# rlabbe/filterpy

Hardware: NVIDIA H100
Metric: kf_predict_update_filter_steps_per_sec (higher is better)
Workload: dtype f32

## Files before the change

filterpy_b200/csrc/kf_fast.cu:

```cuda
#include <string.h>
#include "bke_internal.cuh"
#include "kf_regtile.cuh"
#include "ptx.cuh"

namespace bke {
namespace {

__device__ __forceinline__ void st_hint(float *addr, float4 v, uint64_t pol)
{
    asm volatile("st.global.L2::cache_hint.v4.f32 [%0], {%1, %2, %3, %4}, %5;"
                 ::"l"(addr), "f"(v.x), "f"(v.y), "f"(v.z), "f"(v.w), "l"(pol) : "memory");
}

__device__ __forceinline__ uint32_t ld_relaxed_gpu(const uint32_t *addr)
{
    uint32_t v;
    asm volatile("ld.relaxed.gpu.global.u32 %0, [%1];" : "=r"(v) : "l"(addr) : "memory");
    return v;
}
__device__ __forceinline__ uint32_t atom_add_acq_rel_gpu(uint32_t *addr, uint32_t v)
{
    uint32_t old;
    asm volatile("atom.add.acq_rel.gpu.global.u32 %0, [%1], %2;" : "=r"(old) : "l"(addr), "r"(v) : "memory");
    return old;
}

constexpr int TILE = 128;

constexpr int SYM_Q_PLANES = 10, SYM_PLANES = 13;

constexpr int WORDS = BKE_KF42_MODEL_WORDS, W_F = 0, W_Q = 16, W_H = 26, W_R = 34;
constexpr uint64_t PREDICT_WORDS = (1ull << W_H) - 1;
constexpr int REC_RUNS = (WORDS + 1) / 2;
constexpr int q_word(int i, int j)
{
    const int r = i < j ? i : j, c = i < j ? j : i;
    return W_Q + r * 4 - r * (r - 1) / 2 + (c - r);
}

template <uint64_t Z, uint64_t O>
struct WordPattern {
    static constexpr uint64_t ZERO = Z, ONE = O;
    static constexpr bool any = (ZERO | ONE) != 0;
    static constexpr bool structural(int e) { return ((Z | O) >> e) & 1; }
    static constexpr uint32_t F0(int i) { return (uint32_t)(Z >> (W_F + 4 * i)) & 15u; }
    static constexpr uint32_t F1(int i) { return (uint32_t)(O >> (W_F + 4 * i)) & 15u; }
    static constexpr uint32_t H0(int a) { return (uint32_t)(Z >> (W_H + 4 * a)) & 15u; }
    static constexpr uint32_t H1(int a) { return (uint32_t)(O >> (W_H + 4 * a)) & 15u; }
    static constexpr bool Q0(int i, int j) { return (Z >> q_word(i, j)) & 1; }
    static constexpr bool R0(int a, int b) { return (Z >> (W_R + a + b)) & 1; }
};
struct NoPattern : WordPattern<0, 0> {};
struct Cv2dPattern : WordPattern<
    (1ull << 2) | (1ull << 3) | (1ull << 4) | (1ull << 6) | (1ull << 7) | (1ull << 8) | (1ull << 9) | (1ull << 12) |
        (1ull << 13) | (1ull << 14) | (1ull << q_word(0, 2)) | (1ull << q_word(0, 3)) | (1ull << q_word(1, 2)) |
        (1ull << q_word(1, 3)) | (1ull << 27) | (1ull << 28) | (1ull << 29) | (1ull << 30) | (1ull << 31) |
        (1ull << 33) | (1ull << (W_R + 1)),
    (1ull << 0) | (1ull << 5) | (1ull << 10) | (1ull << 15) | (1ull << 26) | (1ull << 32)> {};

template <typename T, int N, int M, bool SHARED = false, int REC = 0, int ZS = 1>
struct Stage {
    static constexpr int XB = TILE * N * sizeof(T);
    static constexpr int PB = TILE * N * N * sizeof(T);
    static constexpr int HB = TILE * M * N * sizeof(T);
    static constexpr int RB = TILE * M * M * sizeof(T);
    static constexpr int ZB = TILE * M * sizeof(T);
    static constexpr int QB = REC == 1 ? TILE * SYM_PLANES * sizeof(T) : REC == 2 ? TILE * WORDS * sizeof(T) : PB;
    static constexpr int align_up(int v) { return (v + 127) & ~127; }
    static constexpr int OP = 0;
    static constexpr int OF = OP + align_up(PB);
    static constexpr int OQ = OF + (SHARED || REC == 2 ? 0 : align_up(PB));
    static constexpr int OH = OQ + (SHARED ? 0 : align_up(QB));
    static constexpr int OX = OH + (SHARED || REC == 2 ? 0 : align_up(HB));
    static constexpr int OR_ = OX + align_up(XB);
    static constexpr int OZ = OR_ + (SHARED || REC ? 0 : align_up(RB));
    static constexpr int BYTES = OZ + ZS * align_up(ZB);
};

template <int ROWB>
__device__ __forceinline__ float4 lds_chunk(const unsigned char *base, int row, int c)
{
    return *reinterpret_cast<const float4 *>(base + row * ROWB + c * 16);
}

template <int ROWS>
__device__ __forceinline__ void lds_row(const unsigned char *base, int row, float (&m)[ROWS][4])
{
    const int r = (row / (8 / ROWS)) & (ROWS - 1);
    float4 v[ROWS];
#pragma unroll
    for (int c = 0; c < ROWS; c++)
        v[c] = *reinterpret_cast<const float4 *>(base + row * ROWS * 16 + ((c + r) & (ROWS - 1)) * 16);
#pragma unroll
    for (int step = 1; step < ROWS; step <<= 1) {
        const bool rot = r & step;
        float4 w[ROWS];
#pragma unroll
        for (int i = 0; i < ROWS; i++) {
            const float4 a = v[i], b = v[(i - step) & (ROWS - 1)];
            w[i] = make_float4(rot ? b.x : a.x, rot ? b.y : a.y, rot ? b.z : a.z, rot ? b.w : a.w);
        }
#pragma unroll
        for (int i = 0; i < ROWS; i++) v[i] = w[i];
    }
#pragma unroll
    for (int i = 0; i < ROWS; i++) { m[i][0] = v[i].x; m[i][1] = v[i].y; m[i][2] = v[i].z; m[i][3] = v[i].w; }
}

template <int N, int M>
struct FastP {
    int64_t N_filters;
    int num_tiles;
    int l2_hints;
    int reverse;
    float alpha_sq;
    const float *x, *P, *z;
    const float *F, *Q, *H, *R;
    const float *rec;
    float Fh[N * N], Qh[N * N], Hh[M * N], Rh[M * M];
    float *x_out, *P_out;
    const uint8_t *valid;
    float *x_prior, *P_prior, *K, *y, *S, *SI, *ll;
    int32_t *status;
    int sticky;
    uint64_t varying;
    int slot_off[WORDS];
    int rec_planes;
    int rec_copy;
    int rec_runs;
    int run_first[REC_RUNS], run_len[REC_RUNS];
    const float *zs[BKE_KF42_MAX_RING];
    int n_steps;
    int ring_ox, ring_oz, ring_stage;
    uint32_t *order;
};

constexpr int STAGES = 2;
constexpr int kf42_ctas_per_sm(int shared, int ring = 0) { return ring ? 4 : shared == 2 ? 5 : (shared ? 4 : 3); }

template <int MODE, int SHARED, bool EXTRAS, int REC = 0, int RING = 0, class PAT = NoPattern>
__global__ void __launch_bounds__(TILE, kf42_ctas_per_sm(SHARED, RING))
kf42_f32_kernel(const __grid_constant__ FastP<4, 2> p)
{
    constexpr int N = 4, M = 2;
    static_assert(!(REC && SHARED), "the packed records hold per-filter models");
    static_assert(!RING || (MODE == 3 && REC == 2 && !EXTRAS), "the fused ring steps the packed model words");
    static_assert(!PAT::any || RING, "a pattern instance is a fused ring");
    constexpr int ZS = RING ? RING : 1;
    using St = Stage<float, N, M, SHARED != 0, REC, ZS>;
    constexpr int SYM_FIRST = (MODE & 1) ? 0 : SYM_Q_PLANES;
    constexpr int SYM_LAST = (MODE & 2) ? SYM_PLANES : SYM_Q_PLANES;
    constexpr uint32_t SYM_BYTES = (SYM_LAST - SYM_FIRST) * TILE * 4;
    constexpr bool DO_P = MODE & 1, DO_U = MODE & 2;
    extern __shared__ __align__(128) unsigned char smem[];
    __shared__ __align__(8) uint64_t full[STAGES];

    const int tid = threadIdx.x;
    const int stage_bytes = RING ? p.ring_stage : St::BYTES, off_x = RING ? p.ring_ox : St::OX,
              off_z = RING ? p.ring_oz : St::OZ;

    const uint64_t pol_first = policy_evict_first(), pol_last = policy_evict_last();
    auto issue = [&](int tile, int stage) {
        unsigned char *sb = smem + stage * stage_bytes;
        uint64_t *bar = &full[stage];
        const int64_t f0 = (int64_t)tile * TILE;
        const int64_t left = p.N_filters - f0;
        const uint32_t nf = left < TILE ? (uint32_t)left : (uint32_t)TILE;
        const uint32_t zb = (nf * M * 4) & ~15u;
        uint32_t tx = nf * (N + N * N) * 4;
        if (!SHARED && REC != 2 && DO_P) tx += nf * (REC ? 1 : 2) * N * N * 4;
        if (!SHARED && REC != 2 && DO_U) tx += nf * (M * N + (REC ? 0 : M * M)) * 4;
        if (REC == 1) tx += SYM_BYTES;
        if (REC == 2) tx += (uint32_t)p.rec_copy * TILE * 4;
        if (DO_U) tx += RING ? p.n_steps * zb : zb;
        mbar_expect_tx(bar, tx);
        auto load = [&](int off, const float *src, int per_filter, uint32_t bytes, uint64_t pol) {
            if (p.l2_hints) bulk_load_hint(sb + off, src + f0 * per_filter, bytes, bar, pol);
            else bulk_load(sb + off, src + f0 * per_filter, bytes, bar);
        };
        load(St::OP, p.P, N * N, nf * N * N * 4, pol_last);
        load(off_x, p.x, N, nf * N * 4, pol_last);
        if (!SHARED && REC != 2 && DO_P) {
            load(St::OF, p.F, N * N, nf * N * N * 4, pol_first);
            if (!REC) load(St::OQ, p.Q, N * N, nf * N * N * 4, pol_first);
        }
        if (!SHARED && REC != 2 && DO_U) {
            load(St::OH, p.H, M * N, nf * M * N * 4, pol_first);
            if (!REC) load(St::OR_, p.R, M * M, nf * M * M * 4, pol_first);
        }
        if (REC == 1) load(St::OQ + SYM_FIRST * TILE * 4, p.rec + SYM_FIRST * TILE, SYM_PLANES, SYM_BYTES, pol_first);
        if (REC == 2)
            for (int r = 0; r < p.rec_runs; r++)
                load(St::OQ + p.run_first[r] * TILE * 4, p.rec + p.run_first[r] * TILE, p.rec_planes,
                     p.run_len[r] * TILE * 4, pol_first);
        if (!RING && DO_U && zb) load(St::OZ, p.z, M, zb, pol_first);
        if (RING && zb)
            for (int k = 0; k < p.n_steps; k++) load(off_z + k * St::align_up(St::ZB), p.zs[k], M, zb, pol_first);
    };

    if (tid == 0) {
        for (int s = 0; s < STAGES; s++) mbar_init(&full[s], 1);
        fence_mbar_init();
    }
    float F[N][N], Q[N][N], H[M][N], R[M][M];
    if (SHARED == 2) {
#pragma unroll
        for (int i = 0; i < N; i++)
#pragma unroll
            for (int j = 0; j < N; j++) { F[i][j] = p.Fh[i * N + j]; Q[i][j] = p.Qh[i * N + j]; }
#pragma unroll
        for (int a = 0; a < M; a++) {
#pragma unroll
            for (int j = 0; j < N; j++) H[a][j] = p.Hh[a * N + j];
#pragma unroll
            for (int b = 0; b < M; b++) R[a][b] = p.Rh[a * M + b];
        }
    }
    griddep_wait();
    __shared__ uint32_t order_epoch;
    if (RING && p.order && tid == 0) order_epoch = ld_relaxed_gpu(p.order);
    __syncthreads();
    const int reverse = RING && p.order ? (int)(order_epoch & 1u) : p.reverse;
    const int base = reverse ? p.num_tiles - 1 : 0, sign = reverse ? -1 : 1;
    if (tid == 0) {
        for (int s = 0; s < STAGES; s++) {
            int tile = blockIdx.x + s * gridDim.x;
            if (tile < p.num_tiles) issue(base + sign * tile, s);
        }
    }
    if (SHARED == 1) {
        if (DO_P) {
#pragma unroll
            for (int i = 0; i < N; i++)
#pragma unroll
                for (int j = 0; j < N; j++) { F[i][j] = __ldg(p.F + i * N + j); Q[i][j] = __ldg(p.Q + i * N + j); }
        }
        if (DO_U) {
#pragma unroll
            for (int a = 0; a < M; a++) {
#pragma unroll
                for (int j = 0; j < N; j++) H[a][j] = __ldg(p.H + a * N + j);
#pragma unroll
                for (int b = 0; b < M; b++) R[a][b] = __ldg(p.R + a * M + b);
            }
        }
    }

    int it = 0;
    for (int tile = blockIdx.x; tile < p.num_tiles; tile += gridDim.x, it++) {
        const int stage = it % STAGES;
        const uint32_t parity = (it / STAGES) & 1;
        const unsigned char *sb = smem + stage * stage_bytes;
        mbar_wait(&full[stage], parity);

        float x[N], P[N][N], z[ZS][M];
        {
            float4 v = lds_chunk<16>(sb + off_x, tid, 0);
            x[0] = v.x; x[1] = v.y; x[2] = v.z; x[3] = v.w;
        }
        lds_row<N>(sb + St::OP, tid, P);
        const unsigned char *rec = sb + St::OQ + tid * 4;
        auto word = [&](int e, float shared) -> float {
            if (PAT::structural(e)) return (PAT::ONE >> e) & 1 ? 1.f : 0.f;
            if (REC == 1) return *reinterpret_cast<const float *>(rec + (e < W_H ? e - W_Q : e - W_R + SYM_Q_PLANES) * TILE * 4);
            return (p.varying >> e) & 1 ? *reinterpret_cast<const float *>(rec + p.slot_off[e]) : shared;
        };
        if (!SHARED && DO_P) {
            if (REC == 2) {
#pragma unroll
                for (int i = 0; i < N; i++)
#pragma unroll
                    for (int j = 0; j < N; j++) F[i][j] = word(W_F + i * N + j, p.Fh[i * N + j]);
            } else {
                lds_row<N>(sb + St::OF, tid, F);
            }
            if (REC) {
                int k = W_Q;
#pragma unroll
                for (int i = 0; i < N; i++)
#pragma unroll
                    for (int j = i; j < N; j++, k++) Q[i][j] = Q[j][i] = word(k, p.Qh[i * N + j]);
            } else {
                lds_row<N>(sb + St::OQ, tid, Q);
            }
        }
        if (!SHARED && DO_U) {
            if (REC == 2) {
#pragma unroll
                for (int a = 0; a < M; a++)
#pragma unroll
                    for (int j = 0; j < N; j++) H[a][j] = word(W_H + a * N + j, p.Hh[a * N + j]);
            } else {
                lds_row<M>(sb + St::OH, tid, H);
            }
            if (REC) {
                R[0][0] = word(W_R, p.Rh[0]);
                R[0][1] = R[1][0] = word(W_R + 1, p.Rh[1]);
                R[1][1] = word(W_R + 2, p.Rh[3]);
            } else {
                float4 r = lds_chunk<16>(sb + St::OR_, tid, 0);
                R[0][0] = r.x; R[0][1] = r.y; R[1][0] = r.z; R[1][1] = r.w;
            }
        }
        const int64_t f = (int64_t)(base + sign * tile) * TILE + tid;
        const bool live = f < p.N_filters;
        if (DO_U) {
            const bool own = live && (p.N_filters & 1) && f == p.N_filters - 1;
            if (!RING) {
                float2 v = own ? *reinterpret_cast<const float2 *>(p.z + f * M)
                               : *reinterpret_cast<const float2 *>(sb + St::OZ + tid * 8);
                z[0][0] = v.x; z[0][1] = v.y;
            }
#pragma unroll
            for (int k = 0; k < RING; k++) {
                float2 v = make_float2(0.f, 0.f);
                if (k < p.n_steps)
                    v = own ? *reinterpret_cast<const float2 *>(p.zs[k] + f * M)
                            : *reinterpret_cast<const float2 *>(sb + off_z + k * St::align_up(St::ZB) + tid * 8);
                z[k][0] = v.x; z[k][1] = v.y;
            }
        }
        unsigned acc = 0;
#pragma unroll
        for (int i = 0; i < N; i++) {
            acc ^= __float_as_uint(x[i]);
#pragma unroll
            for (int j = 0; j < N; j++) acc ^= __float_as_uint(P[i][j]);
        }
        if (!SHARED && DO_P) {
#pragma unroll
            for (int i = 0; i < N; i++)
#pragma unroll
                for (int j = 0; j < N; j++) {
                    if (!PAT::structural(W_F + i * N + j)) acc ^= __float_as_uint(F[i][j]);
                    if ((!REC || j >= i) && !PAT::structural(q_word(i, j))) acc ^= __float_as_uint(Q[i][j]);
                }
        }
        if (!SHARED && DO_U) {
#pragma unroll
            for (int a = 0; a < M; a++) {
#pragma unroll
                for (int j = 0; j < N; j++)
                    if (!PAT::structural(W_H + a * N + j)) acc ^= __float_as_uint(H[a][j]);
#pragma unroll
                for (int b = 0; b < M; b++)
                    if ((!REC || b >= a) && !PAT::structural(W_R + a + b)) acc ^= __float_as_uint(R[a][b]);
            }
        }
        if (DO_U) {
#pragma unroll
            for (int k = 0; k < ZS; k++) acc ^= __float_as_uint(z[k][0]) ^ __float_as_uint(z[k][1]);
        }
        const int never = __syncthreads_and(acc == 0x7fc0beefu);
        if (never && p.num_tiles < 0) p.x_out[0] = 0.f;
        const int nt = tile + STAGES * gridDim.x;
        if (nt < p.num_tiles) {
            if (tid == 0) issue(base + sign * nt, stage);
        } else {
            griddep_launch_dependents();
        }

        int st = BKE_STATUS_OK;
        if (RING) {
            float nf = 0.f;
            auto check = [&](float v) { nf = __fmaf_rn(0.f, v, nf); };
            if (PAT::any) {
                check(p.alpha_sq);
#pragma unroll
                for (int i = 0; i < N; i++) {
                    check(x[i]);
#pragma unroll
                    for (int j = 0; j < N; j++) {
                        check(P[i][j]);
                        if (!PAT::structural(W_F + i * N + j)) check(F[i][j]);
                        if (j >= i && !PAT::structural(q_word(i, j))) check(Q[i][j]);
                    }
                }
#pragma unroll
                for (int a = 0; a < M; a++) {
#pragma unroll
                    for (int j = 0; j < N; j++)
                        if (!PAT::structural(W_H + a * N + j)) check(H[a][j]);
#pragma unroll
                    for (int b = a; b < M; b++)
                        if (!PAT::structural(W_R + a + b)) check(R[a][b]);
                }
#pragma unroll
                for (int k = 0; k < ZS; k++) { check(z[k][0]); check(z[k][1]); }
            }
#pragma unroll 1
            for (int k = 0; k < p.n_steps; k++) {
                if (PAT::any) {
                    reg_predict_pat<PAT, N>(x, P, F, Q, p.alpha_sq);
                    reg_update_pat<PAT, N, M>(x, P, H, R, z[0]);
                } else {
                    reg_predict<float, N>(x, P, F, Q, p.alpha_sq);
                    KfUpdateOut<float, N, M> o;
                    reg_update<float, N, M>(x, P, H, R, z[0], o);
                }
#pragma unroll
                for (int j = 0; j + 1 < ZS; j++) { z[j][0] = z[j + 1][0]; z[j][1] = z[j + 1][1]; }
            }
            if (PAT::any) {
#pragma unroll
                for (int i = 0; i < N; i++) {
                    check(x[i]);
#pragma unroll
                    for (int j = 0; j < N; j++) check(P[i][j]);
                }
            }
            if (PAT::any && live && nf != 0.f) {
                const float *rec = p.rec + (int64_t)(base + sign * tile) * p.rec_planes * TILE + tid;
                auto gword = [&](int e, float shared) -> float {
                    if (PAT::structural(e)) return shared;
                    return (p.varying >> e) & 1 ? rec[p.slot_off[e] / 4] : shared;
                };
                float Fd[N][N], Qd[N][N], Hd[M][N], Rd[M][M];
#pragma unroll
                for (int i = 0, e = W_Q; i < N; i++) {
#pragma unroll
                    for (int j = 0; j < N; j++) Fd[i][j] = gword(W_F + i * N + j, p.Fh[i * N + j]);
#pragma unroll
                    for (int j = i; j < N; j++, e++) Qd[i][j] = Qd[j][i] = gword(e, p.Qh[i * N + j]);
                }
#pragma unroll
                for (int a = 0; a < M; a++)
#pragma unroll
                    for (int j = 0; j < N; j++) Hd[a][j] = gword(W_H + a * N + j, p.Hh[a * N + j]);
                Rd[0][0] = gword(W_R, p.Rh[0]);
                Rd[0][1] = Rd[1][0] = gword(W_R + 1, p.Rh[1]);
                Rd[1][1] = gword(W_R + 2, p.Rh[3]);
                const float4 vx = *reinterpret_cast<const float4 *>(p.x + f * N);
                x[0] = vx.x; x[1] = vx.y; x[2] = vx.z; x[3] = vx.w;
#pragma unroll
                for (int i = 0; i < N; i++) {
                    const float4 v = *reinterpret_cast<const float4 *>(p.P + f * N * N + i * N);
                    P[i][0] = v.x; P[i][1] = v.y; P[i][2] = v.z; P[i][3] = v.w;
                }
#pragma unroll 1
                for (int k = 0; k < p.n_steps; k++) {
                    const float2 v = *reinterpret_cast<const float2 *>(p.zs[k] + f * M);
                    const float zk[M] = {v.x, v.y};
                    reg_predict<float, N>(x, P, Fd, Qd, p.alpha_sq);
                    KfUpdateOut<float, N, M> o;
                    reg_update<float, N, M>(x, P, Hd, Rd, zk, o);
                }
            }
        }
        if (!RING && DO_P) {
            reg_predict<float, N>(x, P, F, Q, p.alpha_sq);
            if (EXTRAS && live) {
                if (p.x_prior) *reinterpret_cast<float4 *>(p.x_prior + f * N) = make_float4(x[0], x[1], x[2], x[3]);
                if (p.P_prior) {
#pragma unroll
                    for (int i = 0; i < N; i++)
                        *reinterpret_cast<float4 *>(p.P_prior + f * N * N + i * N) = make_float4(P[i][0], P[i][1], P[i][2], P[i][3]);
                }
            }
        }
        if (!RING && DO_U) {
            bool has_z = true;
            if (p.valid != nullptr && live) has_z = p.valid[f] != 0;
            KfUpdateOut<float, N, M> o;
            if (has_z) {
                reg_update<float, N, M>(x, P, H, R, z[0], o);
                if (!o.ok) st = BKE_STATUS_SINGULAR_S;
            }
            if (EXTRAS && live) {
                if (!has_z) {
                    if (p.y) *reinterpret_cast<float2 *>(p.y + f * M) = make_float2(0.f, 0.f);
                } else {
                    if (p.S) *reinterpret_cast<float4 *>(p.S + f * M * M) = make_float4(o.S[0][0], o.S[0][1], o.S[1][0], o.S[1][1]);
                    if (o.ok) {
                        if (p.y) *reinterpret_cast<float2 *>(p.y + f * M) = make_float2(o.y[0], o.y[1]);
                        if (p.SI) *reinterpret_cast<float4 *>(p.SI + f * M * M) = make_float4(o.SI[0][0], o.SI[0][1], o.SI[1][0], o.SI[1][1]);
                        if (p.K) {
                            *reinterpret_cast<float4 *>(p.K + f * N * M) = make_float4(o.K[0][0], o.K[0][1], o.K[1][0], o.K[1][1]);
                            *reinterpret_cast<float4 *>(p.K + f * N * M + 4) = make_float4(o.K[2][0], o.K[2][1], o.K[3][0], o.K[3][1]);
                        }
                        if (p.ll) {
                            float q = 0.f;
#pragma unroll
                            for (int a = 0; a < M; a++) {
                                float s = 0.f;
#pragma unroll
                                for (int b = 0; b < M; b++) s += o.SI[a][b] * o.y[b];
                                q += o.y[a] * s;
                            }
                            p.ll[f] = -0.5f * (q + o.logdet + float(M) * float(LOG_2PI));
                        }
                    }
                }
            }
        }
        if (live) {
            if (p.l2_hints) {
                st_hint(p.x_out + f * N, make_float4(x[0], x[1], x[2], x[3]), pol_last);
#pragma unroll
                for (int i = 0; i < N; i++)
                    st_hint(p.P_out + f * N * N + i * N, make_float4(P[i][0], P[i][1], P[i][2], P[i][3]), pol_last);
            } else {
                *reinterpret_cast<float4 *>(p.x_out + f * N) = make_float4(x[0], x[1], x[2], x[3]);
#pragma unroll
                for (int i = 0; i < N; i++)
                    *reinterpret_cast<float4 *>(p.P_out + f * N * N + i * N) = make_float4(P[i][0], P[i][1], P[i][2], P[i][3]);
            }
            if (EXTRAS && p.status && (st != BKE_STATUS_OK || !p.sticky)) p.status[f] = st;
        }
    }
    if (RING && p.order && tid == 0) {
        if (atom_add_acq_rel_gpu(p.order + 1, 1u) == gridDim.x - 1) {
            p.order[1] = 0u;
            p.order[0] = order_epoch + 1u;
        }
    }
}

template <int MODE, int SHARED, bool EXTRAS, int REC = 0, int RING = 0, class PAT = NoPattern>
int launch_variant(const FastP<4, 2> &p, cudaStream_t s)
{
    using St = Stage<float, 4, 2, SHARED != 0, REC, RING ? RING : 1>;
    auto kern = kf42_f32_kernel<MODE, SHARED, EXTRAS, REC, RING, PAT>;
    const int smem = STAGES * (RING ? p.ring_stage : St::BYTES);
    static bool configured[64] = {false};
    int dev = 0;
    cudaGetDevice(&dev);
    if (dev < 0 || dev >= 64 || !configured[dev]) {
        if (check_cuda(cudaFuncSetAttribute(kern, cudaFuncAttributeMaxDynamicSharedMemorySize, STAGES * St::BYTES),
                       "cudaFuncSetAttribute")) return BKE_ERR_CUDA;
        if (dev >= 0 && dev < 64) configured[dev] = true;
    }
    int ctas = kf42_ctas_per_sm(SHARED, RING);
    if (RING) {
        constexpr int UNITS = STAGES * St::BYTES / 512 + 1;
        static int resident[64][UNITS] = {};
        const int unit = smem / 512;
        int *r = dev >= 0 && dev < 64 && unit < UNITS ? &resident[dev][unit] : nullptr;
        if (!r || *r == 0) {
            int n = 0;
            if (check_cuda(cudaOccupancyMaxActiveBlocksPerMultiprocessor(&n, kern, TILE, smem), "cudaOccupancyMaxActiveBlocksPerMultiprocessor"))
                return BKE_ERR_CUDA;
            if (n < 1) n = 1;
            if (r) *r = n;
            ctas = n;
        } else {
            ctas = *r;
        }
    }
    int grid = sm_count() * ctas;
    if (grid > p.num_tiles) grid = p.num_tiles;
    cudaLaunchAttribute attr[1];
    attr[0].id = cudaLaunchAttributeProgrammaticStreamSerialization;
    attr[0].val.programmaticStreamSerializationAllowed = 1;
    cudaLaunchConfig_t cfg = {};
    cfg.gridDim = dim3(grid);
    cfg.blockDim = dim3(TILE);
    cfg.dynamicSmemBytes = smem;
    cfg.stream = s;
    cfg.attrs = attr;
    cfg.numAttrs = 1;
    return check_cuda(cudaLaunchKernelEx(&cfg, kern, p), "kf42_f32_kernel launch");
}

__global__ void __launch_bounds__(256)
kf42_pack_sym_kernel(int64_t n_filters, int64_t slots, const float4 *__restrict__ Q, const float4 *__restrict__ R,
                     float *__restrict__ rec, int32_t *asym)
{
    for (int64_t f = blockIdx.x * (int64_t)blockDim.x + threadIdx.x; f < slots; f += (int64_t)gridDim.x * blockDim.x) {
        float v[SYM_PLANES] = {};
        bool bad = false;
        if (f < n_filters) {
            float q[4][4];
#pragma unroll
            for (int i = 0; i < 4; i++) {
                const float4 r = Q[f * 4 + i];
                q[i][0] = r.x; q[i][1] = r.y; q[i][2] = r.z; q[i][3] = r.w;
            }
            const float4 r = R[f];
            int k = 0;
#pragma unroll
            for (int i = 0; i < 4; i++)
#pragma unroll
                for (int j = i; j < 4; j++, k++) {
                    v[k] = q[i][j];
                    bad |= __float_as_uint(q[i][j]) != __float_as_uint(q[j][i]);
                }
            v[SYM_Q_PLANES] = r.x; v[SYM_Q_PLANES + 1] = r.y; v[SYM_Q_PLANES + 2] = r.w;
            bad |= __float_as_uint(r.y) != __float_as_uint(r.z);
        }
        float *out = rec + (f / TILE) * (SYM_PLANES * TILE) + (f % TILE);
#pragma unroll
        for (int k = 0; k < SYM_PLANES; k++) out[k * TILE] = v[k];
        if (bad) *asym = 1;
    }
}

__device__ __forceinline__ void kf42_model_words(const float4 *__restrict__ F, const float4 *__restrict__ Q,
                                                 const float4 *__restrict__ H, const float4 *__restrict__ R,
                                                 int64_t f, float (&w)[WORDS], bool &asym)
{
    float q[4][4];
#pragma unroll
    for (int i = 0; i < 4; i++) {
        const float4 a = F[f * 4 + i], b = Q[f * 4 + i];
        w[W_F + 4 * i] = a.x; w[W_F + 4 * i + 1] = a.y; w[W_F + 4 * i + 2] = a.z; w[W_F + 4 * i + 3] = a.w;
        q[i][0] = b.x; q[i][1] = b.y; q[i][2] = b.z; q[i][3] = b.w;
    }
    asym = false;
    int k = W_Q;
#pragma unroll
    for (int i = 0; i < 4; i++)
#pragma unroll
        for (int j = i; j < 4; j++, k++) {
            w[k] = q[i][j];
            asym |= __float_as_uint(q[i][j]) != __float_as_uint(q[j][i]);
        }
#pragma unroll
    for (int a = 0; a < 2; a++) {
        const float4 h = H[f * 2 + a];
        w[W_H + 4 * a] = h.x; w[W_H + 4 * a + 1] = h.y; w[W_H + 4 * a + 2] = h.z; w[W_H + 4 * a + 3] = h.w;
    }
    const float4 r = R[f];
    w[W_R] = r.x; w[W_R + 1] = r.y; w[W_R + 2] = r.w;
    asym |= __float_as_uint(r.y) != __float_as_uint(r.z);
}

__global__ void __launch_bounds__(256)
kf42_scan_models_kernel(int64_t n_filters, const float4 *__restrict__ F, const float4 *__restrict__ Q,
                        const float4 *__restrict__ H, const float4 *__restrict__ R, bke_kf_model_map *map)
{
    float w0[WORDS], w[WORDS];
    bool asym = false, a;
    kf42_model_words(F, Q, H, R, 0, w0, a);
    uint32_t lo = 0, hi = 0;
    for (int64_t f = blockIdx.x * (int64_t)blockDim.x + threadIdx.x; f < n_filters; f += (int64_t)gridDim.x * blockDim.x) {
        kf42_model_words(F, Q, H, R, f, w, a);
        asym |= a;
#pragma unroll
        for (int e = 0; e < WORDS; e++) {
            const uint32_t d = __float_as_uint(w[e]) != __float_as_uint(w0[e]);
            if (e < 32) lo |= d << e;
            else hi |= d << (e - 32);
        }
    }
    if (blockIdx.x == 0 && threadIdx.x == 0) {
#pragma unroll
        for (int e = 0; e < WORDS; e++) map->words[e] = w0[e];
    }
    __shared__ uint32_t red[3][8];
    lo = __reduce_or_sync(FULL, lo);
    hi = __reduce_or_sync(FULL, hi);
    const uint32_t as = __reduce_or_sync(FULL, asym ? 1u : 0u);
    const int warp = threadIdx.x / 32, lane = threadIdx.x % 32;
    if (lane == 0) { red[0][warp] = lo; red[1][warp] = hi; red[2][warp] = as; }
    __syncthreads();
    if (threadIdx.x == 0) {
        for (int i = 1; i < (int)blockDim.x / 32; i++) { lo |= red[0][i]; hi |= red[1][i]; }
        uint32_t as_all = 0;
        for (int i = 0; i < (int)blockDim.x / 32; i++) as_all |= red[2][i];
        const unsigned long long v = (unsigned long long)hi << 32 | lo;
        if (v) atomicOr(reinterpret_cast<unsigned long long *>(&map->varying), v);
        if (as_all) atomicOr(&map->asymmetric, 1);
    }
}

__global__ void __launch_bounds__(256)
kf42_scan_duplicates_kernel(int64_t n_filters, const float4 *__restrict__ F, const float4 *__restrict__ Q,
                            const float4 *__restrict__ H, const float4 *__restrict__ R, bke_kf_model_map *map)
{
    __shared__ float col[WORDS][256];
    __shared__ uint8_t pair_e[32], pair_c[32], pair_s[32];
    __shared__ int n_pairs;
    __shared__ uint32_t cand;
    __shared__ uint32_t red[8];
    const int tid = threadIdx.x;
    if (tid == 0) {
        const uint64_t v = map->varying;
        int slot_word[32], n = 0;
        uint32_t c = 0;
        for (int e = 0, s = 0; e < WORDS && s < 32; e++) {
            if (!((v >> e) & 1)) continue;
            slot_word[s] = e;
            for (int t = 0; t < s; t++)
                if (__float_as_uint(map->words[slot_word[t]]) == __float_as_uint(map->words[e])) {
                    pair_e[n] = e; pair_c[n] = slot_word[t]; pair_s[n] = s; n++;
                    c |= 1u << s;
                    break;
                }
            s++;
        }
        n_pairs = n;
        cand = c;
    }
    __syncthreads();
// ... 264 lines not shown
```

filterpy_b200/csrc/kf_regtile.cuh:

```cuda
#pragma once
#include "bke_internal.cuh"

namespace bke {

template <typename T, int N, int M>
struct KfRegs {
    T x[N];
    T P[N][N];
};

template <typename T, int N>
__device__ __forceinline__ void reg_predict(T (&x)[N], T (&P)[N][N], const T (&F)[N][N], const T (&Q)[N][N], T alpha_sq)
{
    T xn[N];
#pragma unroll
    for (int i = 0; i < N; i++) {
        T s = F[i][0] * x[0];
#pragma unroll
        for (int k = 1; k < N; k++) s += F[i][k] * x[k];
        xn[i] = s;
    }
    T FP[N][N];
#pragma unroll
    for (int i = 0; i < N; i++)
#pragma unroll
        for (int j = 0; j < N; j++) {
            T s = F[i][0] * P[0][j];
#pragma unroll
            for (int k = 1; k < N; k++) s += F[i][k] * P[k][j];
            FP[i][j] = s;
        }
#pragma unroll
    for (int i = 0; i < N; i++)
#pragma unroll
        for (int j = 0; j < N; j++) {
            T s = FP[i][0] * F[j][0];
#pragma unroll
            for (int k = 1; k < N; k++) s += FP[i][k] * F[j][k];
            P[i][j] = alpha_sq * s + Q[i][j];
        }
#pragma unroll
    for (int i = 0; i < N; i++) x[i] = xn[i];
}

template <typename T, int M>
__device__ __forceinline__ bool reg_inverse(const T (&S)[M][M], T (&SI)[M][M], T &logdet)
{
    if constexpr (M == 1) {
        logdet = log(fabs(S[0][0]));
        SI[0][0] = T(1) / S[0][0];
        return S[0][0] != T(0);
    } else if constexpr (M == 2) {
        T det = S[0][0] * S[1][1] - S[0][1] * S[1][0];
        T r = T(1) / det;
        SI[0][0] = S[1][1] * r; SI[0][1] = -S[0][1] * r;
        SI[1][0] = -S[1][0] * r; SI[1][1] = S[0][0] * r;
        logdet = log(fabs(det));
        return det != T(0);
    } else {
        T A[M][M];
        bool ok = true;
        T ld = T(0);
#pragma unroll
        for (int i = 0; i < M; i++)
#pragma unroll
            for (int j = 0; j < M; j++) { A[i][j] = S[i][j]; SI[i][j] = (i == j) ? T(1) : T(0); }
#pragma unroll
        for (int c = 0; c < M; c++) {
            T best = fabs(A[c][c]);
#pragma unroll
            for (int r = c + 1; r < M; r++) {
                const T cand = fabs(A[r][c]);
                const bool sw = cand > best;
                best = sw ? cand : best;
#pragma unroll
                for (int j = 0; j < M; j++) {
                    const T a0 = A[c][j], a1 = A[r][j], s0 = SI[c][j], s1 = SI[r][j];
                    A[c][j] = sw ? a1 : a0; A[r][j] = sw ? a0 : a1;
                    SI[c][j] = sw ? s1 : s0; SI[r][j] = sw ? s0 : s1;
                }
            }
            T piv = A[c][c];
            ok = ok && (piv != T(0));
            ld += log(fabs(piv));
            T d = T(1) / piv;
#pragma unroll
            for (int j = 0; j < M; j++) { A[c][j] *= d; SI[c][j] *= d; }
#pragma unroll
            for (int r = 0; r < M; r++) {
                if (r != c) {
                    T f = A[r][c];
#pragma unroll
                    for (int j = 0; j < M; j++) { A[r][j] -= f * A[c][j]; SI[r][j] -= f * SI[c][j]; }
                }
            }
        }
        logdet = ld;
        return ok;
    }
}

template <typename T, int N, int M>
struct KfUpdateOut {
    T y[M];
    T K[N][M];
    T S[M][M];
    T SI[M][M];
    T logdet;
    bool ok;
};

template <typename T, int N, int M, bool RECIP = false>
__device__ __forceinline__ void reg_update(T (&x)[N], T (&P)[N][N], const T (&H)[M][N], const T (&R)[M][M],
                                           const T (&z)[M], KfUpdateOut<T, N, M> &o)
{
    static_assert(!RECIP || M == 1, "the reciprocal gain is the one-row block's");
#pragma unroll
    for (int a = 0; a < M; a++) {
        T s = H[a][0] * x[0];
#pragma unroll
        for (int k = 1; k < N; k++) s += H[a][k] * x[k];
        o.y[a] = z[a] - s;
    }
    T PHT[N][M];
#pragma unroll
    for (int i = 0; i < N; i++)
#pragma unroll
        for (int a = 0; a < M; a++) {
            T s = P[i][0] * H[a][0];
#pragma unroll
            for (int k = 1; k < N; k++) s += P[i][k] * H[a][k];
            PHT[i][a] = s;
        }
#pragma unroll
    for (int a = 0; a < M; a++)
#pragma unroll
        for (int b = 0; b < M; b++) {
            T s = H[a][0] * PHT[0][b];
#pragma unroll
            for (int k = 1; k < N; k++) s += H[a][k] * PHT[k][b];
            o.S[a][b] = s + R[a][b];
        }
    o.ok = reg_inverse<T, M>(o.S, o.SI, o.logdet);
    if (!RECIP && !o.ok) return;
#pragma unroll
    for (int i = 0; i < N; i++)
#pragma unroll
        for (int a = 0; a < M; a++) {
            T s = PHT[i][0] * o.SI[0][a];
#pragma unroll
            for (int b = 1; b < M; b++) s += PHT[i][b] * o.SI[b][a];
            o.K[i][a] = s;
        }
#pragma unroll
    for (int i = 0; i < N; i++) {
        T s = x[i];
#pragma unroll
        for (int a = 0; a < M; a++) s += o.K[i][a] * o.y[a];
        x[i] = s;
    }
    T IKH[N][N];
#pragma unroll
    for (int i = 0; i < N; i++)
#pragma unroll
        for (int j = 0; j < N; j++) {
            T s = (i == j) ? T(1) : T(0);
#pragma unroll
            for (int a = 0; a < M; a++) s -= o.K[i][a] * H[a][j];
            IKH[i][j] = s;
        }
    T T1[N][N];
#pragma unroll
    for (int i = 0; i < N; i++)
#pragma unroll
        for (int j = 0; j < N; j++) {
            T s = IKH[i][0] * P[0][j];
#pragma unroll
            for (int k = 1; k < N; k++) s += IKH[i][k] * P[k][j];
            T1[i][j] = s;
        }
    T KR[N][M];
#pragma unroll
    for (int i = 0; i < N; i++)
#pragma unroll
        for (int b = 0; b < M; b++) {
            T s = o.K[i][0] * R[0][b];
#pragma unroll
            for (int a = 1; a < M; a++) s += o.K[i][a] * R[a][b];
            KR[i][b] = s;
        }
#pragma unroll
    for (int i = 0; i < N; i++)
#pragma unroll
        for (int j = 0; j < N; j++) {
            T s = T1[i][0] * IKH[j][0];
#pragma unroll
            for (int k = 1; k < N; k++) s += T1[i][k] * IKH[j][k];
#pragma unroll
            for (int a = 0; a < M; a++) s += KR[i][a] * o.K[j][a];
            P[i][j] = s;
        }
}

template <typename T, int N, int M>
__device__ __forceinline__ void reg_update_correlated(T (&x)[N], T (&P)[N][N], const T (&H)[M][N], const T (&R)[M][M],
                                                      const T (&Mc)[N][M], const T (&z)[M], KfUpdateOut<T, N, M> &o)
{
#pragma unroll
    for (int a = 0; a < M; a++) {
        T s = H[a][0] * x[0];
#pragma unroll
        for (int k = 1; k < N; k++) s += H[a][k] * x[k];
        o.y[a] = z[a] - s;
    }
    T PHT[N][M], HM[M][M];
#pragma unroll
    for (int i = 0; i < N; i++)
#pragma unroll
        for (int a = 0; a < M; a++) {
            T s = P[i][0] * H[a][0];
#pragma unroll
            for (int k = 1; k < N; k++) s += P[i][k] * H[a][k];
            PHT[i][a] = s;
        }
#pragma unroll
    for (int a = 0; a < M; a++)
#pragma unroll
        for (int b = 0; b < M; b++) {
            T s = H[a][0] * Mc[0][b];
#pragma unroll
            for (int k = 1; k < N; k++) s += H[a][k] * Mc[k][b];
            HM[a][b] = s;
        }
#pragma unroll
    for (int a = 0; a < M; a++)
#pragma unroll
        for (int b = 0; b < M; b++) {
            T s = H[a][0] * PHT[0][b];
#pragma unroll
            for (int k = 1; k < N; k++) s += H[a][k] * PHT[k][b];
            o.S[a][b] = s + HM[a][b] + HM[b][a] + R[a][b];
        }
    o.ok = reg_inverse<T, M>(o.S, o.SI, o.logdet);
    if (!o.ok) return;
#pragma unroll
    for (int i = 0; i < N; i++)
#pragma unroll
        for (int a = 0; a < M; a++) {
            T s = (PHT[i][0] + Mc[i][0]) * o.SI[0][a];
#pragma unroll
            for (int b = 1; b < M; b++) s += (PHT[i][b] + Mc[i][b]) * o.SI[b][a];
            o.K[i][a] = s;
        }
#pragma unroll
    for (int i = 0; i < N; i++) {
        T s = x[i];
#pragma unroll
        for (int a = 0; a < M; a++) s += o.K[i][a] * o.y[a];
        x[i] = s;
    }
    T G[M][N];
#pragma unroll
    for (int a = 0; a < M; a++)
#pragma unroll
        for (int j = 0; j < N; j++) {
            T s = H[a][0] * P[0][j];
#pragma unroll
            for (int k = 1; k < N; k++) s += H[a][k] * P[k][j];
            G[a][j] = s + Mc[j][a];
        }
#pragma unroll
    for (int i = 0; i < N; i++)
#pragma unroll
        for (int j = 0; j < N; j++) {
            T s = o.K[i][0] * G[0][j];
#pragma unroll
            for (int a = 1; a < M; a++) s += o.K[i][a] * G[a][j];
            P[i][j] -= s;
        }
}


template <int L>
__device__ __forceinline__ float and_bits(const float (&b)[L], uint32_t D)
{
    uint32_t m = ~0u;
#pragma unroll
    for (int k = 0; k < L; k++)
        if ((D >> k) & 1) m &= __float_as_uint(b[k]);
    return __uint_as_float(m);
}

template <int L>
__device__ __forceinline__ float pat_chain(uint32_t Z, uint32_t O, bool SIGNED, const float (&a)[L], const float (&b)[L])
{
    float s = 0.f;
    bool have = false;
    uint32_t d = 0;
#pragma unroll
    for (int p = 0; p < L; p++) {
        const int k = L > 1 && p < 2 ? 1 - p : p;
        if ((Z >> k) & 1) {
            if (SIGNED) d |= 1u << k;
            continue;
        }
        const bool one = (O >> k) & 1;
        if (!have) {
            have = true;
            if (one) { s = b[k]; continue; }
            s = d ? __fmaf_rn(a[k], b[k], __fmul_rn(0.f, and_bits(b, d))) : __fmul_rn(a[k], b[k]);
            d = 0;
            continue;
        }
        if (d) { s = __fmaf_rn(0.f, and_bits(b, d), s); d = 0; }
        s = one ? __fadd_rn(s, b[k]) : __fmaf_rn(a[k], b[k], s);
    }
    if (d) s = have ? __fmaf_rn(0.f, and_bits(b, d), s) : __fmul_rn(0.f, and_bits(b, d));
    return s;
}

template <class PAT, int N>
__device__ __forceinline__ void reg_predict_pat(float (&x)[N], float (&P)[N][N], const float (&F)[N][N],
                                                const float (&Q)[N][N], float alpha_sq)
{
    float xn[N];
#pragma unroll
    for (int i = 0; i < N; i++) xn[i] = pat_chain(PAT::F0(i), PAT::F1(i), true, F[i], x);
    float FP[N][N];
#pragma unroll
    for (int j = 0; j < N; j++) {
        float col[N];
#pragma unroll
        for (int k = 0; k < N; k++) col[k] = P[k][j];
#pragma unroll
        for (int i = 0; i < N; i++) FP[i][j] = pat_chain(PAT::F0(i), PAT::F1(i), true, F[i], col);
    }
#pragma unroll
    for (int i = 0; i < N; i++)
#pragma unroll
        for (int j = 0; j < N; j++)
            P[i][j] = __fmaf_rn(alpha_sq, pat_chain(PAT::F0(j), PAT::F1(j), !PAT::Q0(i, j), F[j], FP[i]), Q[i][j]);
#pragma unroll
    for (int i = 0; i < N; i++) x[i] = xn[i];
}

template <class PAT, int M>
__host__ __device__ constexpr uint32_t pat_cols(bool any)
{
    uint32_t c = ~0u;
    for (int a = 0; a < M; a++) c &= any ? PAT::H0(a) | PAT::H1(a) : PAT::H0(a);
    return c;
}

template <class PAT, int N, int M>
__device__ __forceinline__ bool reg_update_pat(float (&x)[N], float (&P)[N][N], const float (&H)[M][N],
                                               const float (&R)[M][M], const float (&z)[M])
{
    float y[M];
#pragma unroll
    for (int a = 0; a < M; a++) y[a] = __fadd_rn(z[a], -pat_chain(PAT::H0(a), PAT::H1(a), true, H[a], x));
    float PHT[N][M];
#pragma unroll
    for (int i = 0; i < N; i++)
#pragma unroll
        for (int a = 0; a < M; a++) PHT[i][a] = pat_chain(PAT::H0(a), PAT::H1(a), true, H[a], P[i]);
    float S[M][M], SI[M][M], logdet;
#pragma unroll
    for (int b = 0; b < M; b++) {
        float col[N];
#pragma unroll
        for (int k = 0; k < N; k++) col[k] = PHT[k][b];
#pragma unroll
        for (int a = 0; a < M; a++) S[a][b] = __fadd_rn(pat_chain(PAT::H0(a), PAT::H1(a), !PAT::R0(a, b), H[a], col), R[a][b]);
    }
    if (!reg_inverse<float, M>(S, SI, logdet)) return false;
    float K[N][M];
#pragma unroll
    for (int i = 0; i < N; i++)
#pragma unroll
        for (int a = 0; a < M; a++) {
            float s = PHT[i][0] * SI[0][a];
#pragma unroll
            for (int b = 1; b < M; b++) s += PHT[i][b] * SI[b][a];
            K[i][a] = s;
        }
#pragma unroll
    for (int i = 0; i < N; i++) {
        float s = x[i];
#pragma unroll
        for (int a = 0; a < M; a++) s += K[i][a] * y[a];
        x[i] = s;
    }
    constexpr uint32_t HS = pat_cols<PAT, M>(true), HZ = pat_cols<PAT, M>(false);
    float IKH[N][N];
#pragma unroll
    for (int j = 0; j < N; j++) {
#pragma unroll
        for (int i = 0; i < N; i++) {
            float s = i == j ? 1.f : 0.f;
            if ((HS >> j) & 1) {
#pragma unroll
                for (int a = 0; a < M; a++)
                    if ((PAT::H1(a) >> j) & 1) s = __fadd_rn(s, -K[i][a]);
            } else {
#pragma unroll
                for (int a = 0; a < M; a++) s = __fmaf_rn(-K[i][a], H[a][j], s);
            }
            IKH[i][j] = s;
        }
    }
    float T1[N][N];
#pragma unroll
    for (int j = 0; j < N; j++) {
        float col[N];
#pragma unroll
        for (int k = 0; k < N; k++) col[k] = P[k][j];
#pragma unroll
        for (int i = 0; i < N; i++) T1[i][j] = pat_chain(HZ & ~(1u << i), HZ & (1u << i), true, IKH[i], col);
    }
    float KR[N][M];
#pragma unroll
    for (int b = 0; b < M; b++) {
        float col[M];
        uint32_t rz = 0;
#pragma unroll
        for (int a = 0; a < M; a++) { col[a] = R[a][b]; rz |= PAT::R0(a, b) ? 1u << a : 0u; }
#pragma unroll
        for (int i = 0; i < N; i++) KR[i][b] = pat_chain(rz, 0u, true, col, K[i]);
    }
#pragma unroll
    for (int j = 0; j < N; j++) {
        float a[N + M];
#pragma unroll
        for (int k = 0; k < N; k++) a[k] = IKH[j][k];
#pragma unroll
        for (int k = 0; k < M; k++) a[N + k] = K[j][k];
#pragma unroll
        for (int i = 0; i < N; i++) {
            float b[N + M];
#pragma unroll
            for (int k = 0; k < N; k++) b[k] = T1[i][k];
#pragma unroll
            for (int k = 0; k < M; k++) b[N + k] = KR[i][k];
            P[i][j] = pat_chain(HZ & ~(1u << j), HZ & (1u << j), true, a, b);
        }
    }
    return true;
}


}
```

Before: 45.24 billion.

## Add block-diagonal fast path for decoupled 2D constant-velocity filter

Adds a specialised predict/update path that runs when the pattern's F, Q, H and R decouple into two 2x2 blocks and a warp-wide check finds the cross-block covariance entries zero. Inside this path the cross-block products are replaced with sign-only zero_chain computations, and the off-diagonal S entries are forced to zero, which removes most of the 4x4 matrix arithmetic. pat_chain and and_bits gain an extra mask argument so that skipped terms still reproduce the exact signed-zero and NaN propagation. The cost is more code size and register pressure, plus a warp vote before the loop.

```diff
diff --git a/filterpy_b200/csrc/kf_fast.cu b/filterpy_b200/csrc/kf_fast.cu
--- a/filterpy_b200/csrc/kf_fast.cu
+++ b/filterpy_b200/csrc/kf_fast.cu
@@ -49,6 +49,16 @@
     static constexpr uint32_t H1(int a) { return (uint32_t)(O >> (W_H + 4 * a)) & 15u; }
     static constexpr bool Q0(int i, int j) { return (Z >> q_word(i, j)) & 1; }
     static constexpr bool R0(int a, int b) { return (Z >> (W_R + a + b)) & 1; }
+    static constexpr bool h_in(int a, int b) { return (H0(a) & blk_other(2 * b)) == blk_other(2 * b); }
+    static constexpr int HB(int a) { return h_in(a, 0) ? 0 : 1; }
+    static constexpr bool blocks()
+    {
+        for (int i = 0; i < 4; i++)
+            for (int k = 0; k < 4; k++)
+                if (blk_cross(i, k) && !(((Z >> (W_F + 4 * i + k)) & 1) && Q0(i, k))) return false;
+        const bool rows = (h_in(0, 0) && h_in(1, 1)) || (h_in(0, 1) && h_in(1, 0));
+        return rows && R0(0, 1);
+    }
 };
 struct NoPattern : WordPattern<0, 0> {};
 struct Cv2dPattern : WordPattern<
@@ -388,8 +398,27 @@
 #pragma unroll
                 for (int k = 0; k < ZS; k++) { check(z[k][0]); check(z[k][1]); }
             }
+            bool blk = false;
+            if constexpr (PAT::blocks()) {
+                uint32_t c = 0;
+#pragma unroll
+                for (int i = 0; i < N; i++)
+#pragma unroll
+                    for (int j = 0; j < N; j++)
+                        if (blk_cross(i, j)) c |= __float_as_uint(P[i][j]);
+                blk = __all_sync(FULL, !live || (c & 0x7fffffffu) == 0);
+                if (blk) {
 #pragma unroll 1
-            for (int k = 0; k < p.n_steps; k++) {
+                    for (int k = 0; k < p.n_steps; k++) {
+                        reg_predict_blk<PAT, N>(x, P, F, Q, p.alpha_sq);
+                        reg_update_blk<PAT, N, M>(x, P, H, R, z[0]);
+#pragma unroll
+                        for (int j = 0; j + 1 < ZS; j++) { z[j][0] = z[j + 1][0]; z[j][1] = z[j + 1][1]; }
+                    }
+                }
+            }
+#pragma unroll 1
+            for (int k = 0; k < (blk ? 0 : p.n_steps); k++) {
                 if (PAT::any) {
                     reg_predict_pat<PAT, N>(x, P, F, Q, p.alpha_sq);
                     reg_update_pat<PAT, N, M>(x, P, H, R, z[0]);
diff --git a/filterpy_b200/csrc/kf_regtile.cuh b/filterpy_b200/csrc/kf_regtile.cuh
--- a/filterpy_b200/csrc/kf_regtile.cuh
+++ b/filterpy_b200/csrc/kf_regtile.cuh
@@ -282,25 +282,40 @@
 
 
 template <int L>
-__device__ __forceinline__ float and_bits(const float (&b)[L], uint32_t D)
+__device__ __forceinline__ float and_bits(const float (&a)[L], const float (&b)[L], uint32_t D, uint32_t X)
 {
     uint32_t m = ~0u;
 #pragma unroll
     for (int k = 0; k < L; k++)
-        if ((D >> k) & 1) m &= __float_as_uint(b[k]);
+        if ((D >> k) & 1) m &= (X >> k) & 1 ? __float_as_uint(a[k]) ^ __float_as_uint(b[k]) : __float_as_uint(b[k]);
     return __uint_as_float(m);
 }
 
 template <int L>
-__device__ __forceinline__ float pat_chain(uint32_t Z, uint32_t O, bool SIGNED, const float (&a)[L], const float (&b)[L])
+__device__ __forceinline__ float pat_chain(uint32_t Z, uint32_t O, bool SIGNED, const float (&a)[L], const float (&b)[L],
+                                           uint32_t X = 0)
 {
     float s = 0.f;
     bool have = false;
     uint32_t d = 0;
+    auto ra = [&](uint32_t r) {
+        float v = 0.f;
+#pragma unroll
+        for (int k = 0; k < L; k++)
+            if (r == (1u << k) && (X >> k) & 1) v = a[k];
+        return v;
+    };
+    auto rb = [&](uint32_t r) {
+        float v = and_bits(a, b, r, X);
+#pragma unroll
+        for (int k = 0; k < L; k++)
+            if (r == (1u << k) && (X >> k) & 1) v = b[k];
+        return v;
+    };
 #pragma unroll
     for (int p = 0; p < L; p++) {
         const int k = L > 1 && p < 2 ? 1 - p : p;
-        if ((Z >> k) & 1) {
+        if (((Z | X) >> k) & 1) {
             if (SIGNED) d |= 1u << k;
             continue;
         }
@@ -308,15 +323,24 @@
         if (!have) {
             have = true;
             if (one) { s = b[k]; continue; }
-            s = d ? __fmaf_rn(a[k], b[k], __fmul_rn(0.f, and_bits(b, d))) : __fmul_rn(a[k], b[k]);
+            s = d ? __fmaf_rn(a[k], b[k], __fmul_rn(ra(d), rb(d))) : __fmul_rn(a[k], b[k]);
             d = 0;
             continue;
         }
-        if (d) { s = __fmaf_rn(0.f, and_bits(b, d), s); d = 0; }
+        if (d) { s = __fmaf_rn(ra(d), rb(d), s); d = 0; }
         s = one ? __fadd_rn(s, b[k]) : __fmaf_rn(a[k], b[k], s);
     }
-    if (d) s = have ? __fmaf_rn(0.f, and_bits(b, d), s) : __fmul_rn(0.f, and_bits(b, d));
+    if (d) s = have ? __fmaf_rn(ra(d), rb(d), s) : __fmul_rn(ra(d), rb(d));
     return s;
+}
+
+template <int L>
+__device__ __forceinline__ float zero_chain(const float (&a)[L], const float (&b)[L])
+{
+    uint32_t m = ~0u;
+#pragma unroll
+    for (int k = 0; k < L; k++) m &= __float_as_uint(a[k]) ^ __float_as_uint(b[k]);
+    return __uint_as_float(m & 0x80000000u);
 }
 
 template <class PAT, int N>
@@ -448,5 +472,140 @@
     return true;
 }
 
-
-}
+__host__ __device__ constexpr bool blk_cross(int i, int j) { return (i >> 1) != (j >> 1); }
+__host__ __device__ constexpr uint32_t blk_other(int i) { return (i >> 1) ? 3u : 12u; }
+
+template <class PAT, int N>
+__device__ __forceinline__ void reg_predict_blk(float (&x)[N], float (&P)[N][N], const float (&F)[N][N],
+                                                const float (&Q)[N][N], float alpha_sq)
+{
+    static_assert(N == 4, "two blocks of two");
+    float xn[N];
+#pragma unroll
+    for (int i = 0; i < N; i++) xn[i] = pat_chain(PAT::F0(i), PAT::F1(i), true, F[i], x);
+    float FP[N][N];
+#pragma unroll
+    for (int j = 0; j < N; j++) {
+        float col[N];
+#pragma unroll
+        for (int k = 0; k < N; k++) col[k] = P[k][j];
+#pragma unroll
+        for (int i = 0; i < N; i++)
+            FP[i][j] = blk_cross(i, j) ? zero_chain(F[i], col) : pat_chain(PAT::F0(i), PAT::F1(i), true, F[i], col);
+    }
+#pragma unroll
+    for (int i = 0; i < N; i++)
+#pragma unroll
+        for (int j = 0; j < N; j++)
+            P[i][j] = blk_cross(i, j) ? 0.f
+                                      : __fmaf_rn(alpha_sq, pat_chain(PAT::F0(j), PAT::F1(j), !PAT::Q0(i, j), F[j], FP[i]), Q[i][j]);
+#pragma unroll
+    for (int i = 0; i < N; i++) x[i] = xn[i];
+}
+
+template <class PAT, int N, int M>
+__device__ __forceinline__ bool reg_update_blk(float (&x)[N], float (&P)[N][N], const float (&H)[M][N],
+                                               const float (&R)[M][M], const float (&z)[M])
+{
+    static_assert(N == 4 && M == 2, "two blocks of two, one measurement row each");
+    float y[M];
+#pragma unroll
+    for (int a = 0; a < M; a++) y[a] = __fadd_rn(z[a], -pat_chain(PAT::H0(a), PAT::H1(a), true, H[a], x));
+    auto hx = [](int i, int a) { return (i >> 1) != PAT::HB(a); };
+    float PHT[N][M];
+#pragma unroll
+    for (int i = 0; i < N; i++)
+#pragma unroll
+        for (int a = 0; a < M; a++)
+            PHT[i][a] = hx(i, a) ? zero_chain(H[a], P[i]) : pat_chain(PAT::H0(a), PAT::H1(a), true, H[a], P[i]);
+    float S[M][M], SI[M][M], logdet;
+#pragma unroll
+    for (int b = 0; b < M; b++) {
+        float col[N];
+#pragma unroll
+        for (int k = 0; k < N; k++) col[k] = PHT[k][b];
+#pragma unroll
+        for (int a = 0; a < M; a++)
+            S[a][b] = a != b ? 0.f : __fadd_rn(pat_chain(PAT::H0(a), PAT::H1(a), !PAT::R0(a, b), H[a], col), R[a][b]);
+    }
+    if (!reg_inverse<float, M>(S, SI, logdet)) return false;
+    float K[N][M];
+#pragma unroll
+    for (int i = 0; i < N; i++)
+#pragma unroll
+        for (int a = 0; a < M; a++) {
+            const float col[M] = {SI[0][a], SI[1][a]};
+            K[i][a] = hx(i, a) ? zero_chain(PHT[i], col) : pat_chain(0u, 0u, true, PHT[i], col, 3u & ~(1u << a));
+        }
+#pragma unroll
+    for (int i = 0; i < N; i++) {
+        float s = x[i];
+#pragma unroll
+        for (int a = 0; a < M; a++) s += K[i][a] * y[a];
+        x[i] = s;
+    }
+    constexpr uint32_t HS = pat_cols<PAT, M>(true), HZ = pat_cols<PAT, M>(false);
+    float IKH[N][N];
+#pragma unroll
+    for (int j = 0; j < N; j++) {
+#pragma unroll
+        for (int i = 0; i < N; i++) {
+            float s = i == j ? 1.f : 0.f;
+            if (blk_cross(i, j)) {
+            } else if ((HS >> j) & 1) {
+#pragma unroll
+                for (int a = 0; a < M; a++)
+                    if ((PAT::H1(a) >> j) & 1) s = __fadd_rn(s, -K[i][a]);
+            } else {
+#pragma unroll
+                for (int a = 0; a < M; a++) s = __fmaf_rn(-K[i][a], H[a][j], s);
+            }
+            IKH[i][j] = s;
+        }
+    }
+    float T1[N][N];
+#pragma unroll
+    for (int j = 0; j < N; j++) {
+        float col[N];
+#pragma unroll
+        for (int k = 0; k < N; k++) col[k] = P[k][j];
+#pragma unroll
+        for (int i = 0; i < N; i++)
+            T1[i][j] = blk_cross(i, j) ? zero_chain(IKH[i], col)
+                                       : pat_chain(HZ & ~(1u << i), HZ & (1u << i), true, IKH[i], col, blk_other(i) & ~HZ);
+    }
+    float KR[N][M];
+#pragma unroll
+    for (int b = 0; b < M; b++) {
+        float col[M];
+        uint32_t rz = 0;
+#pragma unroll
+        for (int a = 0; a < M; a++) { col[a] = R[a][b]; rz |= PAT::R0(a, b) ? 1u << a : 0u; }
+#pragma unroll
+        for (int i = 0; i < N; i++) KR[i][b] = hx(i, b) ? zero_chain(col, K[i]) : pat_chain(rz, 0u, true, col, K[i]);
+    }
+#pragma unroll
+    for (int j = 0; j < N; j++) {
+        float a[N + M];
+#pragma unroll
+        for (int k = 0; k < N; k++) a[k] = IKH[j][k];
+#pragma unroll
+        for (int k = 0; k < M; k++) a[N + k] = K[j][k];
+        uint32_t xj = blk_other(j) & ~HZ;
+#pragma unroll
+        for (int k = 0; k < M; k++) xj |= hx(j, k) ? 1u << (N + k) : 0u;
+#pragma unroll
+        for (int i = 0; i < N; i++) {
+            float b[N + M];
+#pragma unroll
+            for (int k = 0; k < N; k++) b[k] = T1[i][k];
+#pragma unroll
+            for (int k = 0; k < M; k++) b[N + k] = KR[i][k];
+            P[i][j] = blk_cross(i, j) ? zero_chain(a, b) : pat_chain(HZ & ~(1u << j), HZ & (1u << j), true, a, b, xj);
+        }
+    }
+    return true;
+}
+
+
+}
```

Measured after the change: 48.00 billion (median of 6 runs). 1.06x the previous value.
